# METHODS-Group/ProximalGalerkin

Hardware: AMD Instinct MI355X
Metric: proximal-Newton iterations/sec, 2048^2 P1 obstacle (LVPP Newton inner loop) (higher is better)
Workload: dtype f64; 1 GPU; 2048x2048 right-diagonal P1 obstacle problem on [-1,1]^2, phi_set obstacle, f=0, settings B: alpha double_exponential, alpha_max 100, tol 0.0001; snes_rtol 1e-6, Newton linear solves to true relative residual 1e-10; mixed_unknowns=8396802, step=one full LVPP solve from the zero state, parallelism=single

## Files before the change

### include/pgx.h

```cpp
#ifndef PGX_H
#define PGX_H

#include <stdint.h>

#ifdef __cplusplus
extern "C" {
#endif

#define PGX_OK 0
#define PGX_EINVAL (-1)
#define PGX_EHIP (-2)
#define PGX_ENODEV (-3)
#define PGX_ENOMEM (-4)
#define PGX_ESTATE (-5)
#define PGX_ECOMM (-6)

#define PGX_SNES_CONVERGED_FNORM_ABS 2
#define PGX_SNES_CONVERGED_FNORM_RELATIVE 3
#define PGX_SNES_CONVERGED_SNORM_RELATIVE 4
#define PGX_SNES_DIVERGED_LINEAR_SOLVE (-3)
#define PGX_SNES_DIVERGED_FNORM_NAN (-4)
#define PGX_SNES_DIVERGED_MAX_IT (-5)
#define PGX_SNES_DIVERGED_DTOL (-9)

// ... 85 lines not shown

int pgx_umg_level_export(pgx_handle* h, int level, int32_t* n, int32_t* nnz, int32_t* rowptr, int32_t* col, double* K, double* M, double* D,
                         uint8_t* mask);
int pgx_umg_cycle_apply(pgx_handle* h, int level, int nu, double omega, const double* b, double* z);

int pgx_p2_cycle_info(pgx_handle* h, int32_t out[8], double* patch_omega);
int pgx_p2_patch_export(pgx_handle* h, int32_t* pdof, double* Ainv);
int pgx_p2_wide_export(pgx_handle* h, int32_t* nw, int32_t* verts, int32_t* wdof, double* Ainv);
int pgx_p2_cycle_apply(pgx_handle* h, int stage, int nu, double omega, const double* b, const double* x0, double* z);

int pgx_newton_solve(pgx_handle* h, const pgx_snes_opts* opts, int* reason, int* its, int* lin_its);
int pgx_observables(pgx_handle* h, double out[6]);

int pgx_reduce_selfcheck(pgx_handle* h, int nv, int64_t len, int basis_f32, int reps, uint64_t seed, int64_t* mismatches);

int pgx_profile_enable(pgx_handle* h, int on);
int pgx_profile_get(pgx_handle* h, double ms[8], int reset);

typedef struct pgx_comm pgx_comm;

typedef struct pgx_partition {
  int32_t rank, size;
  int32_t global_ny;
  int32_t dist_levels;
} pgx_partition;

int pgx_partition_rows(pgx_partition* part, int32_t* row0, int32_t* nrows, int32_t* own0, int32_t* nown);

int pgx_comm_rccl_unique_id(char id[128]);
int pgx_comm_rccl_init(const char id[128], int rank, int size, int device, pgx_comm** out);
// ... 23 lines not shown
```

### proximalgalerkin_amd/_lib.py

```python
from __future__ import annotations

import ctypes as C
import pathlib

import numpy as np

_HERE = pathlib.Path(__file__).resolve().parent
import os as _os

LIB_PATH = pathlib.Path(_os.environ.get("PGX_LIB", _HERE / "libpgx.so"))

c_double_p = C.POINTER(C.c_double)
c_int32_p = C.POINTER(C.c_int32)
c_int64_p = C.POINTER(C.c_int64)


class PgxError(RuntimeError):
    pass


class pgx_mesh(C.Structure):
    _fields_ = [
        ("n_vertices", C.c_int32),
        ("n_cells", C.c_int32),
# ... 345 lines not shown
    ("pgx_umg_transfer_export", C.c_int, [_H, C.c_int, c_int32_p, c_int32_p, c_int32_p, c_int32_p, c_int32_p, c_double_p]),
    ("pgx_umg_level_export", C.c_int,
     [_H, C.c_int, c_int32_p, c_int32_p, c_int32_p, c_int32_p, c_double_p, c_double_p, c_double_p, C.POINTER(C.c_uint8)]),
    ("pgx_umg_cycle_apply", C.c_int, [_H, C.c_int, C.c_int, C.c_double, c_double_p, c_double_p]),
    ("pgx_p2_cycle_info", C.c_int, [_H, c_int32_p, c_double_p]),
    ("pgx_p2_patch_export", C.c_int, [_H, c_int32_p, c_double_p]),
    ("pgx_p2_wide_export", C.c_int, [_H, c_int32_p, c_int32_p, c_int32_p, c_double_p]),
    ("pgx_p2_cycle_apply", C.c_int, [_H, C.c_int, C.c_int, C.c_double, c_double_p, c_double_p, c_double_p]),
    ("pgx_spmv_select", C.c_int, [_H, C.c_int, C.POINTER(C.c_int)]),
    ("pgx_p2_stencil_info", C.c_int, [_H, C.POINTER(C.c_int32)]),
    ("pgx_comm_counts", C.c_int, [_H, C.POINTER(C.c_int64), C.c_int]),
    ("pgx_newton_solve", C.c_int,
     [_H, C.POINTER(pgx_snes_opts), C.POINTER(C.c_int), C.POINTER(C.c_int), C.POINTER(C.c_int)]),
    ("pgx_observables", C.c_int, [_H, c_double_p]),
    ("pgx_reduce_selfcheck", C.c_int, [_H, C.c_int, C.c_int64, C.c_int, C.c_int, C.c_uint64, c_int64_p]),
    ("pgx_profile_enable", C.c_int, [_H, C.c_int]),
    ("pgx_profile_get", C.c_int, [_H, c_double_p, C.c_int]),
    ("pgx_partition_rows", C.c_int,
     [C.POINTER(pgx_partition), c_int32_p, c_int32_p, c_int32_p, c_int32_p]),
    ("pgx_comm_rccl_unique_id", C.c_int, [C.c_char_p]),
    ("pgx_comm_rccl_init", C.c_int, [C.c_char_p, C.c_int, C.c_int, C.c_int, C.POINTER(_COMM)]),
    ("pgx_comm_local_group", C.c_int, [C.c_int, C.POINTER(_COMM)]),
    ("pgx_comm_shm_init", C.c_int, [C.c_char_p, C.c_int, C.c_int, C.c_uint64, C.c_int, C.POINTER(_COMM)]),
    ("pgx_comm_allreduce", C.c_int, [_COMM, c_double_p, C.c_uint64]),
    ("pgx_comm_halo", C.c_int, [_COMM, c_double_p, c_double_p] + [C.c_uint64] * 8),
    ("pgx_comm_gather0", C.c_int, [_COMM, c_double_p, C.c_uint64, c_double_p]),
    ("pgx_comm_scatter0", C.c_int, [_COMM, c_double_p, C.c_uint64, c_double_p]),
    ("pgx_comm_selfcheck", C.c_int, [_COMM, C.c_int, C.c_double]),
    ("pgx_comm_free", None, [_COMM]),
    ("pgx_comm_last_error", C.c_char_p, []),
# ... 225 lines not shown
```

### proximalgalerkin_amd/csrc/pgx_api.hip

```cpp
#include <algorithm>
#include <atomic>
#include <chrono>
#include <thread>
#include <cmath>
#include <cstdio>
#include <cstring>
#include <deque>
#include <map>
#include <mutex>
#include <string>
#include <vector>

#include "../../include/pgx.h"
#include "../../include/pgx_nd.h"
#include "pgx_comm.h"
#include "pgx_handle.h"
#include "pgx_internal.h"

static thread_local std::string g_create_error;

namespace {
std::mutex g_tune_mu;
std::atomic<int> g_tune_gen{0};
std::map<std::string, const std::string*>& tune_table() {
// ... 931 lines not shown
  if (!h->patch_f32) h->patch_sym = 0;
  if (h->patch_f32 == 2 && !h->patch_sym) h->patch_f32 = 1;
  if (const char* e = pgx_tune("PGX_P2_FALLBACK_ITS")) h->p2_fallback_its = std::max(1, atoi(e));
  {
    const char* e = pgx_tune("PGX_TAIL2");
    pgxk_mg_tail_select(e ? atoi(e) : 1);
  }
  if (const char* e = pgx_tune("PGX_FUSED_LEGS")) h->fused_legs = atoi(e);
  if (const char* e = pgx_tune("PGX_FUSED_K3")) h->fused_k3 = atoi(e);
  if (const char* e = pgx_tune("PGX_NU_COARSE")) h->nu_coarse = atoi(e);
  if (const char* e = pgx_tune("PGX_SPMV_STREAM")) h->spmv_stream = atoi(e);
  if (const char* e = pgx_tune("PGX_SPMV_BAL")) h->spmv_bal = atoi(e);
  if (const char* e = pgx_tune("PGX_SPMV_DICT")) h->spmv_dict = atoi(e);
  if (const char* e = pgx_tune("PGX_SPMV_STENCIL")) h->spmv_stencil = atoi(e);
  if (const char* e = pgx_tune("PGX_RESID_GRID")) h->resid_grid = atoi(e);
  if (const char* e = pgx_tune("PGX_D_DIRECT")) h->d_direct = atoi(e);
  if (const char* e = pgx_tune("PGX_RAP_LDS_MIN")) h->rap_lds_min = atoi(e);
  if (const char* e = pgx_tune("PGX_K6_MAX")) h->k6_max = atoi(e);
  if (const char* e = pgx_tune("PGX_SMOOTH_D32")) h->smooth_d32 = atoi(e);
  if (const char* e = pgx_tune("PGX_HOST_POLL")) h->host_poll = atoi(e);
  if (const char* e = pgx_tune("PGX_GS_WIDE")) h->gs_wide = atoi(e) >= 16 ? 16 : 8;
  if (const char* e = pgx_tune("PGX_FUSED_PUBLISH")) h->fused_publish = atoi(e);
  if (const char* e = pgx_tune("PGX_TICKET_REDUCE")) h->ticket_reduce = atoi(e);
  if (const char* e = pgx_tune("PGX_FUSED_RESID")) h->fused_resid = atoi(e);
  if (const char* e = pgx_tune("PGX_LEAN_RHS")) h->lean_rhs = atoi(e);
  if (const char* e = pgx_tune("PGX_FUSED_STEP")) h->fused_step = atoi(e);
  if (const char* e = pgx_tune("PGX_LAZY_NORM")) h->lazy_norm = atoi(e);
  if (const char* e = pgx_tune("PGX_V_F32")) h->v_f32 = atoi(e);
  if (const char* e = pgx_tune("PGX_V_F32_GAIN")) h->v_f32_gain = atof(e);
  if (const char* e = pgx_tune("PGX_V_F32_MAX")) h->v_f32_max = atof(e);
// ... 360 lines not shown
  HIPCHK(hipMemcpyAsync(dst, src, sizeof(double) * 2 * (size_t)h->nd, hipMemcpyHostToDevice, h->st));
  HIPCHK(hipStreamSynchronize(h->st));
  return PGX_OK;
}
static int copy_out(pgx_handle* h, double* dst, const double* src) {
  HIPCHK(hipMemcpyAsync(dst, src, sizeof(double) * 2 * (size_t)h->nd, hipMemcpyDeviceToHost, h->st));
  HIPCHK(hipStreamSynchronize(h->st));
  return PGX_OK;
}
extern "C" int pgx_set_state(pgx_handle* h, const double* x) {
  NEED(h);
  if (!x) return PGX_EINVAL;
  return copy_in(h, h->x, x);
}
extern "C" int pgx_get_state(pgx_handle* h, double* x) {
  NEED(h);
  if (!x) return PGX_EINVAL;
  return copy_out(h, x, h->x);
}
extern "C" int pgx_set_prev(pgx_handle* h, const double* x) {
  NEED(h);
  if (!x) return PGX_EINVAL;
  return copy_in(h, h->xk, x);
}
extern "C" int pgx_get_prev(pgx_handle* h, double* x) {
  NEED(h);
  if (!x) return PGX_EINVAL;
  return copy_out(h, x, h->xk);
}
extern "C" int pgx_advance_prev(pgx_handle* h) {
  NEED(h);
  pgxk_scale_copy(h->st, 2 * (size_t)h->nd, 1.0, h->x, h->xk);
  HIPCHK(hipStreamSynchronize(h->st));
  return PGX_OK;
}
extern "C" int pgx_zero_state(pgx_handle* h) {
  NEED(h);
  HIPCHK(hipMemsetAsync(h->x, 0, sizeof(double) * 2 * (size_t)h->nd, h->st));
  HIPCHK(hipMemsetAsync(h->xk, 0, sizeof(double) * 2 * (size_t)h->nd, h->st));
  HIPCHK(hipStreamSynchronize(h->st));
  return PGX_OK;
}
extern "C" int pgx_owned_range(const pgx_handle* h, int64_t* offset, int64_t* count) {
  if (!h) return PGX_EINVAL;
  if (offset) *offset = h->dist.on ? (int64_t)h->dist.own_off : 0;
  if (count) *count = h->dist.on ? (int64_t)h->dist.own_cnt : (int64_t)(h->degree == 2 ? h->n : h->nd);
// ... 13 lines not shown
  if (rc) return rc;
  HIPCHK(hipStreamSynchronize(h->st));
  return PGX_OK;
}
extern "C" int pgx_set_alpha(pgx_handle* h, double a) {
  if (!h || !(a > 0.0)) return PGX_EINVAL;
  h->alpha = a;
  return PGX_OK;
}

static bool d_direct_on(const pgx_handle* h) {
  return h->d_direct && !h->dist.on && h->degree == 1 && h->structured && h->resid_grid && !h->lev.empty() && h->lev[0].uniform &&
         sizeof(dsten_t) == 8 && !h->lev[0].Dh32;
}

static void residual_dev(pgx_handle* h, const double* x, double* F, int with_d = 0) {
  PhaseTimer t(h, 0);
  if (h->degree == 2) {
    pgxk_residual_p2_cells(h->st, h->nc, h->nd, h->cdofs, h->coords, h->mask, h->gbc, x, h->xk, h->alpha, h->f, h->q2,
                           h->p2_v2c_ptr, h->p2_v2c_ent, h->p2_stash, F, h->geoq);
    pgxk_residual_final(h->st, h->nd, h->mask, h->gbc, h->bphi, x, F);
    return;
  }
  if (h->resid_grid && h->structured && !h->lev.empty() && h->lev[0].uniform) {
    pgxk_resid_fill_grid(h->st, with_d ? 1 : 0, h->lev[0], h->fill_lds, h->rowptr, h->v2c_ptr, h->v2c_ent, h->v2c_pos, h->cells,
                         h->coords, h->mask, h->gbc, h->bphi, x, h->xk, h->alpha, h->f, h->q, F, h->Dv, with_d, d_direct_on(h), h->colm);
    h->dh_interior = with_d != 0;
    h->d0_direct = with_d != 0 && d_direct_on(h);
    if (with_d == 2) h->dv_lean = true;
    if (with_d == 1) h->dv_lean = false;
    return;
  }
  pgxk_resid_fill_p1(h->st, with_d, h->n, h->fill_lds, h->rowptr, h->v2c_ptr, h->v2c_ent, h->v2c_pos, h->cells,
                     h->coords, h->mask, h->gbc, h->bphi, x, h->xk, h->alpha, h->f, h->q, F, h->Dv, h->geoq);
}

static int jacobian_dev(pgx_handle* h, const double* x, bool have_d = false) {
  if (!(have_d && h->degree == 1)) {
    PhaseTimer t(h, 1);
    if (h->degree == 2) {
      pgxk_fill_rows_p2(h->st, 2, h->nd, h->s_fill_lds, h->s_rowptr, h->p2_v2c_ptr, h->p2_v2c_ent, h->p2_v2c_pos,
                        h->cdofs, h->coords, x + h->nd, h->q2, h->s_D, h->geoq);
      pgxk_fill_rows_p1_Dp2(h->st, h->n, h->fill_lds, h->rowptr, h->v2c_ptr, h->v2c_ent, h->v2c_pos, h->cdofs, h->coords,
                            x + h->nd, h->q2, h->Dv, h->geoq);
    } else if (h->resid_grid && h->structured && !h->lev.empty() && h->lev[0].uniform) {
      pgxk_resid_fill_grid(h->st, 1, h->lev[0], h->fill_lds, h->rowptr, h->v2c_ptr, h->v2c_ent, h->v2c_pos, h->cells, h->coords,
                           h->mask, h->gbc, h->bphi, x, h->xk, h->alpha, h->f, h->q, h->w, h->Dv, 1, d_direct_on(h), h->colm);
      h->dh_interior = true;
      h->d0_direct = d_direct_on(h);
      h->dv_lean = false;
      have_d = true;
    } else {
      pgxk_fill_rows(h->st, 2, h->n, h->fill_lds, h->rowptr, h->v2c_ptr, h->v2c_ent, h->v2c_pos, h->cells, h->coords,
                     x + h->n, h->q, h->Dv, h->geoq);
    }
  }
  if (h->structured) {
    PhaseTimer t(h, 2);
    const bool direct = d_direct_on(h);
    const bool d0 = direct && have_d && h->dh_interior && h->d0_direct;
// ... 1602 lines not shown
  NEED(h);
  if (h->degree == 2) {
    if (kind == 0) h->p2st.select = 0;
    else if (kind == 1 || kind == 3) h->p2st.select = 1;
    else if (kind != -1) return PGX_EINVAL;
    if (active) *active = (h->p2st.state && h->p2st.select && (!h->dist.on || h->p2st.dist_enable) && h->spmv_stream && h->spmv_bal) ? 3 : 0;
    return PGX_OK;
  }
  if (kind == 0 || kind == 1 || kind == 2) h->spmv_stencil = kind;
  else if (kind != -1) return PGX_EINVAL;
  if (active) *active = (h->spmv_stencil && h->structured && h->degree == 1) ? h->spmv_stencil : 0;
  return PGX_OK;
}

extern "C" int pgx_observables(pgx_handle* h, double out[6]) {
  NEED(h);
  if (!out) return PGX_EINVAL;
  {
    PhaseTimer t(h, 6);
    if (h->degree == 2 && !h->dist.on) {
      pgxk_observables_p2_cells(h->st, h->nc, h->nd, h->cdofs, h->coords, h->x, h->xk, h->alpha, h->f, h->q2,
                                h->obs_partials, h->obs_blocks, h->geoq);
      pgxk_observables_final(h->st, h->obs_blocks, h->obs_partials, h->d_out6);
    } else if (h->dist.on && h->degree == 2) {
      const Dist& D = h->dist;
      pgxk_observables_p2_cells(h->st, D.ncell_own, h->nd, h->cdofs + 6 * (size_t)D.cell0, h->coords, h->x, h->xk, h->alpha, h->f,
                                h->q2, h->obs_partials, pgxk_observables_blocks(D.ncell_own));
      pgxk_observables_final_raw(h->st, pgxk_observables_blocks(D.ncell_own), h->obs_partials, h->d_out6);
      const int rc = allreduce_dev(h, h->d_out6, 6);
      if (rc) return rc;
    } else if (h->dist.on) {
// ... 13 lines not shown
    if (rcb) return rcb;
  }
  {
    const int rcf = fetch_small(h, h->d_out6, 6);
    if (rcf) return rcf;
  }
  for (int k = 0; k < 6; ++k) out[k] = h->h_small[k];
  if (h->dist.on) {
    out[1] = std::fabs(out[1]);
    out[4] = std::sqrt(out[4]);
    out[5] = std::sqrt(out[5]);
  }
  return PGX_OK;
}

extern "C" int pgx_profile_enable(pgx_handle* h, int on) {
  if (!h) return PGX_EINVAL;
  h->prof = on != 0;
  return PGX_OK;
}
extern "C" int pgx_profile_get(pgx_handle* h, double ms[8], int reset) {
  if (!h || !ms) return PGX_EINVAL;
  for (int k = 0; k < 8; ++k) ms[k] = h->ms[k];
  if (reset)
    for (int k = 0; k < 8; ++k) h->ms[k] = 0.0;
  return PGX_OK;
}

extern "C" int pgx_newton_solve(pgx_handle* h, const pgx_snes_opts* opts, int* reason, int* its_out, int* lin_out) {
  NEED(h);
  if (!opts || !reason) return PGX_EINVAL;
  pgx_snes_opts optv = *opts;
  if (!(optv.ksp_rtol > 0.0)) optv.ksp_rtol = (h->degree == 2) ? 1e-11 : 1e-10;
  opts = &optv;
  const bool p2_hier = h->structured ? h->lev.size() > 1 : (umg_on(h) && h->n >= h->umg_min_p2);
  const bool mg_first = optv.pc_type == 0 && h->degree == 2 && p2_hier && h->patch_nn && h->p2_patch && !h->dist.on && !h->lu_comm;
  const bool umg_auto = h->degree == 1 && umg_on(h) && h->n >= h->umg_min;
  bool use_lu = h->lu_comm || optv.pc_type == 2 ||
                (optv.pc_type == 0 && (h->degree == 2 || !h->structured) && !h->dist.on && !mg_first && !umg_auto);
  h->lu_active = false;
  if (use_lu) {
    int rcl = ensure_lu(h);
    if (rcl) return rcl;
  }
  if (h->dist.on && h->degree == 2 && optv.ksp_max_it == 200) optv.ksp_max_it = 400;
// ... 9 lines not shown
  h->umg_idle = use_lu;
  PgxRange range("pgx:newton_solve");
  int its = 0, lin = 0, rsn = 0;
  double fnorm = 0, fnorm0 = 0, ttol = 0;
  h->omega_now = 0.0;
  h->v_f32_off = false;
  int rc = PGX_OK;
  const bool dist = h->dist.on;
  const size_t nk = dist ? 2 * h->dist.nk_field() : n2;
  auto owned_norm = [&](const double* v, double* out) -> int {
    if (!dist) return dev_norm(h, v, out);
    gather_owned(h, v, h->dist.wc);
    return dev_norm(h, h->dist.wc, out, nk);
  };
  const int with_d = (!use_lu && !mg_first && h->degree == 1 && h->structured && h->spmv_stencil == 1 && h->lean_d) ? 2 : 1;
  pgxk_scale_copy(h->st, n2, 1.0, h->x, h->xw);
  residual_dev(h, h->xw, h->F, with_d);
  if ((rc = replica_check(h, h->F, n2, "the residual"))) return rc;
  if (dist) {
    gather_owned(h, h->F, h->rhs);
    rc = dev_norm(h, h->rhs, &fnorm, nk);
  } else {
    rc = dev_norm(h, h->F, &fnorm);
  }
  if (rc) return rc;
  fnorm0 = fnorm;
  if (opts->monitor) printf("  0 SNES Function norm %.12e\n", fnorm);
  if (!std::isfinite(fnorm))
    rsn = PGX_SNES_DIVERGED_FNORM_NAN;
  else if (fnorm < opts->snes_atol)
    rsn = PGX_SNES_CONVERGED_FNORM_ABS;
  ttol = fnorm * opts->snes_rtol;
// ... 80 lines not shown
        if (rc) return rc;
        rc = owned_norm(h->xw, &xnorm);
        if (rc) return rc;
      }
      if (snorm < opts->snes_stol * xnorm)
        rsn = PGX_SNES_CONVERGED_SNORM_RELATIVE;
      else if (fnorm > opts->snes_divtol * fnorm0)
        rsn = PGX_SNES_DIVERGED_DTOL;
    }
  }
  h->lu_active = false;
  if (rsn > 0) pgxk_scale_copy(h->st, n2, 1.0, h->xw, h->x);
  if (h->dh_interior || h->dv_lean) h->jac_valid = false;
  HIPCHK(hipStreamSynchronize(h->st));
  HIPCHK(hipGetLastError());
  if (h->prof) h->ms[7] += scope.stop();
  *reason = rsn;
  if (its_out) *its_out = its;
  if (lin_out) *lin_out = lin;
  return PGX_OK;
}
```

### proximalgalerkin_amd/csrc/pgx_handle.h

```cpp
#pragma once
#include <algorithm>
#include <string>
#include <vector>

#include "../../include/pgx.h"
#include "../../include/pgx_nd.h"
#include "pgx_comm.h"
#include "pgx_internal.h"

struct DistLevel {
  int g, glo, H, ghi;
};
struct Dist {
  bool on = false;
  pgx_comm* comm = nullptr;
  int rank = 0, size = 1, ldist = 0, global_ny = 0;
  std::vector<DistLevel> L;
  GridLevel view{};
  int view_row0 = 0, view_glo = 0, view_H = 0, view_own0 = 0;
  long long n_halo = 0, n_allreduce = 0, n_vcycle = 0, n_krylov = 0;
  double* view_S = nullptr;
  size_t own_off = 0, own_cnt = 0;
  size_t eb = 0, eown_off = 0, eown_cnt = 0;
  size_t nk_field() const { return own_cnt + eown_cnt; }
// ... 146 lines not shown
  pgx_comm* lu_comm = nullptr;
  double* Jmix = nullptr;
  bool dh_interior = false;
  int d_direct = 1;
  int rap_lds_min = 60000;
  bool d0_direct = false;
  int stag_its = 12;
  double stag_gain = 1e-4;
  int smooth_d32 = 0;
  int k6_max = 0;
  int mg_f32 = 1;
  int f32_min = 4000;
  int f32_k6_max = 4300000;
  int f32_rr_max = 300000;
  int resid_grid = 1;
  int spmv_stencil = 1;
  bool lu_active = false;
  bool check_replicas = false;
  double *obs_partials = nullptr, *d_out6 = nullptr;
  int obs_blocks = 0;
  bool prof = false;
  double ms[8] = {0, 0, 0, 0, 0, 0, 0, 0};
  hipEvent_t e0 = nullptr, e1 = nullptr;
  std::vector<void*> allocs;
};

static inline bool umg_on(const pgx_handle* h) { return h->umg.size() > 1 && h->umg_enable; }

#define HIPCHK(call)                                                                           \
  do {                                                                                          \
// ... 63 lines not shown
    pgx_roctx(names[s & 7]);
    if (h->prof) hipEventRecord(h->e0, h->st);
  }
  ~PhaseTimer() {
    pgx_roctx(nullptr);
    if (h->prof) {
      hipEventRecord(h->e1, h->st);
      hipEventSynchronize(h->e1);
      float ms = 0;
      hipEventElapsedTime(&ms, h->e0, h->e1);
      h->ms[slot] += ms;
    }
  }
};

#define NEED(hh)          \
  if (!(hh)) return PGX_EINVAL; \
  hipSetDevice((hh)->device)

#pragma GCC visibility push(hidden)
int precond(pgx_handle* h, const double* b, double* z, int nu, double omega);
void spmv_dev(pgx_handle* h, const double* x, double* y);
void gather_owned(pgx_handle* h, const double* loc, double* cmp);
int allreduce_dev(pgx_handle* h, double* dev, size_t n);
bool f32_cycle_ok(const pgx_handle* h, int l, int nu);

void pgxk_amg_direct(hipStream_t st, int n, const int32_t* ptr, const int32_t* src, const double* K, double* val);
void pgxk_amg_pvalues(hipStream_t st, int n, const int32_t* fptr, const int32_t* own, const int32_t* pptr, const int32_t* pa, const int32_t* pb,
                      const int32_t* diag, const double* K, const double* p0, double trunc, double* val);
int pgx_amg_build_device(pgx_handle* h, double theta, double trunc, int32_t min_coarse, double max_keep, int32_t* n_levels, double* seconds);
void pgxk_amg_rap(hipStream_t st, const UmgLevel& C, const double* src, double* dst);
void pgxk_amg_resid_restrict(hipStream_t st, const UmgLevel& C, const double* ru, const double* rp);
void pgxk_amg_prolong_add(hipStream_t st, int n_f, const UmgLevel& C, double* xu, double* xp);
// ... 52 lines not shown
```

### proximalgalerkin_amd/csrc/pgx_internal.h

```cpp
#pragma once
#include <hip/hip_runtime.h>
#include <stdint.h>
#include <stddef.h>

#include "pgx_scope.h"

#ifdef PGX_DSTEN_FLOAT
typedef float dsten_t;
#else
typedef double dsten_t;
#endif

#define PGX_MAX_NQ 16
#define PGX_BLOCK 256
#ifndef PGX_TILE_X
#define PGX_TILE_X 32
#define PGX_TILE_Y 16
#endif
#ifndef PGX_ROWMAP_TY
#define PGX_ROWMAP_TY 16
#endif
#ifndef PGX_ROWMAP_BLOCK
#define PGX_ROWMAP_BLOCK 512
#endif
// ... 229 lines not shown
                    void* Dst, int f32);
void pgxk_p2st_check(hipStream_t st, const P2StTab& S, int nx, int nv, int i0, int ni, int j0, int nj, double alpha_ref, double tol,
                     const int32_t* rowptr, const double* K, const double* M, int* fail);
void pgxk_p2_rows_csr(hipStream_t st, int nrows, const int32_t* rows, const int32_t* rowptr, const int32_t* colm, const double* K,
                      const double* M, const double* D, double alpha, const uint8_t* mask, const double* xu, const double* xp,
                      const double* bu, const double* bp, double* yu, double* yp);
void pgxk_resid_fill_p1(hipStream_t st, int write_d, int n, size_t lds_bytes, const int32_t* rowptr,
                        const int32_t* v2c_ptr, const int32_t* v2c_ent, const int32_t* v2c_pos, const int32_t* cells,
                        const double* coords, const uint8_t* mask, const double* gbc, const double* bphi,
                        const double* x, const double* xk, double alpha, double f, QuadTab q, double* F, double* Dout,
                        const double* geo = nullptr);
void pgxk_resid_fill_grid(hipStream_t st, int write_d, const GridLevel& L, size_t lds_bytes, const int32_t* rowptr,
                          const int32_t* v2c_ptr, const int32_t* v2c_ent, const int32_t* v2c_pos, const int32_t* cells,
                          const double* coords, const uint8_t* mask, const double* gbc, const double* bphi, const double* x,
                          const double* xk, double alpha, double f, QuadTab q, double* F, double* Dout, int write_sh,
                          int direct = 0, const int32_t* colm = nullptr);
void pgxk_multiaxpy_scale(hipStream_t st, size_t len, int nv, const double* V, size_t ldv, const double* h,
                          double scale, double* w);
bool pgxk_multiaxpy_norm(hipStream_t st, size_t len, int nv, const double* V, size_t ldv, const double* h, double* w,
                         double* partials, double* out, int wide = 8, PgxTicket* tk = nullptr);
bool pgxk_multiaxpy_norm_f32(hipStream_t st, size_t len, int nv, const float* V, size_t ldv, const double* h, int from_vnext, double* w,
                             float* vnext, double* partials, double* out, int wide = 8, PgxTicket* tk = nullptr);
void pgxk_f_pack_d(hipStream_t st, const GridLevel& L);
void pgxk_f_smooth(hipStream_t st, int K, int first, const GridLevel& L, double alpha, const float2* xf, const double* b64u,
                   const double* b64p, const GridLevel* C, const float2* cf, const double* cdu, const double* cdp, double omega,
                   int remap, float2* yf, double* y64u, double* y64p, float2* cbf = nullptr, double* cb64u = nullptr,
                   double* cb64p = nullptr, double bscale = 1.0,
                   const float* b32u = nullptr, const float* b32p = nullptr);
void pgxk_f_resid_restrict(hipStream_t st, const GridLevel& L, double alpha, const float2* xf, const GridLevel& C, int remap,
                           float2* cbf, double* cb64u, double* cb64p);
int pgxk_st_smooth6_ok(const GridLevel& L);
// ... 4 lines not shown
```

### proximalgalerkin_amd/csrc/pgx_kernels.hip

```cpp
#include "pgx_internal.h"
#include "pgx_stencil.h"
#include <algorithm>
#include <type_traits>

#define WAVE 64

static bool first_use_on_device(int slot) {
  static bool done[4][64] = {};
  int dev = 0;
  if (hipGetDevice(&dev) != hipSuccess || dev < 0 || dev >= 64) return true;
  if (done[slot][dev]) return false;
  done[slot][dev] = true;
  return true;
}

__device__ __forceinline__ double wave_sum(double v) {
#pragma unroll
  for (int o = WAVE / 2; o > 0; o >>= 1) v += __shfl_xor(v, o, WAVE);
  return v;
}

__device__ __forceinline__ double2 ldnt2(const double2* p) {
  typedef double v2d __attribute__((ext_vector_type(2)));
  const v2d v = __builtin_nontemporal_load((const v2d*)p);
// ... 413 lines not shown
      }
    }
    F[i] = mask[i] ? x[i] - gbc[i] : Fu;
    F[n + i] = Fp - bphi[i];
    if (WRITE_D && FRAME)
      for (int k = rowptr[i]; k < rowptr[i + 1]; ++k) Dout[k] = row[k - rowptr[i]];
  }
  if (WRITE_D && !FRAME) {
    __syncthreads();
    for (int k = threadIdx.x; k < len; k += PGX_BLOCK) Dout[base + k] = acc[k];
  }
}

#define PGX_RF_TX 32
#define PGX_RF_TY 12
template <bool WRITE_D>
__global__ void __launch_bounds__(PGX_RF_TX * PGX_RF_TY) k_resid_fill_grid(
    int nx, int ny, int n, const int32_t* __restrict__ rowptr, const double* __restrict__ coords, const uint8_t* __restrict__ mask,
    const double* __restrict__ gbc, const double* __restrict__ bphi, const double* __restrict__ x, const double* __restrict__ xk,
    double alpha, double f, QuadTab q, StConst sc, double* __restrict__ F, double* __restrict__ Dout,
    dsten_t* __restrict__ Sh, double4* __restrict__ Dd4, void* __restrict__ Dq, int dbf16) {
  constexpr int TX = PGX_RF_TX, TY = PGX_RF_TY, IW = TX + 2, IH = TY + 2, SW = TX + 1, SH = TY + 1;
  __shared__ double iu[IH * IW], ip[IH * IW], idp[IH * IW];
  __shared__ double E[2 * SW * SH][6];
  const int sx = nx + 1;
  const int ntx = (nx - 1 + TX - 1) / TX;
  const int i1 = 1 + ((int)blockIdx.x % ntx) * TX, j1 = 1 + ((int)blockIdx.x / ntx) * TY;
  const int tid = threadIdx.x;
  for (int t = tid; t < IH * IW; t += TX * TY) {
    const int gi = i1 - 1 + t % IW, gj = j1 - 1 + t / IW;
    double u = 0.0, p = 0.0, dp = 0.0;
    if (gi <= nx && gj <= ny) {
      const int v = gj * sx + gi;
      u = mask[v] ? gbc[v] : x[v];
      p = x[n + v];
      dp = p - xk[n + v];
    }
    iu[t] = u;
    ip[t] = p;
    idp[t] = dp;
  }
  __syncthreads();
  for (int t = tid; t < 2 * SW * SH; t += TX * TY) {
    const int sq = t >> 1, a = sq % SW, b = sq / SW;
    double e[6] = {0.0, 0.0, 0.0, 0.0, 0.0, 0.0};
    if (i1 - 1 + a < nx && j1 - 1 + b < ny) {
      const int o = b * IW + a;
      const double p0 = ip[o], p1 = (t & 1) ? ip[o + IW + 1] : ip[o + 1], p2 = (t & 1) ? ip[o + IW] : ip[o + IW + 1];
      for (int k = 0; k < q.nq; ++k) {
        const double n0 = q.N[k][0], n1 = q.N[k][1], n2 = q.N[k][2];
        const double w = q.w[k] * exp(p0 * n0 + p1 * n1 + p2 * n2);
        e[0] += w * n0 * n0;
        e[1] += w * n1 * n1;
        e[2] += w * n2 * n2;
        e[3] += w * n0 * n1;
        e[4] += w * n0 * n2;
        e[5] += w * n1 * n2;
// ... 166 lines not shown
                         bphi, x, xk, alpha, f, q, F, Dout, geo);
    return;
  }
  if (write_d)
    hipLaunchKernelGGL((k_resid_fill_p1<true, false>), grid, block, lds_bytes, st, n, rowptr, v2c_ptr, v2c_ent, v2c_pos, cells,
                       coords, mask, gbc, bphi, x, xk, alpha, f, q, 0, 0, F, Dout);
  else
    hipLaunchKernelGGL((k_resid_fill_p1<false, false>), grid, block, lds_bytes, st, n, rowptr, v2c_ptr, v2c_ent, v2c_pos, cells,
                       coords, mask, gbc, bphi, x, xk, alpha, f, q, 0, 0, F, Dout);
}

void pgxk_resid_fill_grid(hipStream_t st, int write_d, const GridLevel& L, size_t lds_bytes, const int32_t* rowptr,
                          const int32_t* v2c_ptr, const int32_t* v2c_ent, const int32_t* v2c_pos, const int32_t* cells,
                          const double* coords, const uint8_t* mask, const double* gbc, const double* bphi, const double* x,
                          const double* xk, double alpha, double f, QuadTab q, double* F, double* Dout, int write_sh, int direct,
                          const int32_t* colm) {
  const int n = L.n, sx = L.nx + 1;
  const bool copies = direct && write_d && write_sh && colm;
  double4* Dd4 = copies ? L.Dd4 : nullptr;
  void* Dq = copies && L.f32 ? L.Dq : nullptr;
  if (direct && colm) {
    const int nframe = 2 * sx + 2 * (L.ny - 1);
    dim3 grid((nframe + PGX_FRAME_BLOCK - 1) / PGX_FRAME_BLOCK), block(PGX_FRAME_BLOCK);
    if (write_d)
      hipLaunchKernelGGL(k_resid_fill_frame<true>, grid, block, 0, st, L.nx, L.ny, n, rowptr, colm, v2c_ptr, v2c_ent, v2c_pos, cells,
                         coords, mask, gbc, bphi, x, xk, alpha, f, q, F, Dout, copies ? L.Dh : nullptr, Dd4, Dq, L.dbf16);
    else
      hipLaunchKernelGGL(k_resid_fill_frame<false>, grid, block, 0, st, L.nx, L.ny, n, rowptr, colm, v2c_ptr, v2c_ent, v2c_pos, cells,
                         coords, mask, gbc, bphi, x, xk, alpha, f, q, F, Dout, nullptr, nullptr, nullptr, 0);
  } else {
    dim3 grid((n + PGX_BLOCK - 1) / PGX_BLOCK), block(PGX_BLOCK);
    if (write_d)
      hipLaunchKernelGGL((k_resid_fill_p1<true, true>), grid, block, lds_bytes, st, n, rowptr, v2c_ptr, v2c_ent, v2c_pos, cells,
                         coords, mask, gbc, bphi, x, xk, alpha, f, q, sx, L.ny, F, Dout);
    else
      hipLaunchKernelGGL((k_resid_fill_p1<false, true>), grid, block, lds_bytes, st, n, rowptr, v2c_ptr, v2c_ent, v2c_pos, cells,
                         coords, mask, gbc, bphi, x, xk, alpha, f, q, sx, L.ny, F, Dout);
  }
  if (L.nx < 2 || L.ny < 2) return;
  const int ntx = (L.nx - 1 + PGX_RF_TX - 1) / PGX_RF_TX, nty = (L.ny - 1 + PGX_RF_TY - 1) / PGX_RF_TY;
  const StConst sc = make_stconst(L);
  if (write_d)
    hipLaunchKernelGGL(k_resid_fill_grid<true>, dim3(ntx * nty), dim3(PGX_RF_TX * PGX_RF_TY), 0, st, L.nx, L.ny, n, rowptr, coords,
                       mask, gbc, bphi, x, xk, alpha, f, q, sc, F, write_sh == 2 ? nullptr : Dout, write_sh ? L.Dh : nullptr, Dd4, Dq,
                       L.dbf16);
  else
    hipLaunchKernelGGL(k_resid_fill_grid<false>, dim3(ntx * nty), dim3(PGX_RF_TX * PGX_RF_TY), 0, st, L.nx, L.ny, n, rowptr, coords,
                       mask, gbc, bphi, x, xk, alpha, f, q, sc, F, Dout, nullptr, nullptr, nullptr, 0);
}

void pgxk_fill_rows(hipStream_t st, int mode, int n, size_t lds_bytes, const int32_t* rowptr, const int32_t* v2c_ptr,
                    const int32_t* v2c_ent, const int32_t* v2c_pos, const int32_t* cells, const double* coords,
                    const double* psi, QuadTab q, double* out, const double* geo) {
  dim3 grid((n + PGX_BLOCK - 1) / PGX_BLOCK), block(PGX_BLOCK);
  if (geo) {
    if (mode == 0)
      hipLaunchKernelGGL(k_fill_rows_c<0>, grid, block, lds_bytes, st, n, rowptr, v2c_ptr, v2c_ent, v2c_pos, cells, psi, q, out, geo);
// ... 3199 lines not shown
```

### proximalgalerkin_amd/problem.py

```python
from __future__ import annotations

import ctypes as C
import warnings
from dataclasses import dataclass

import numpy as np

from . import _lib
from .fem import Constant, DirichletBC, Function, QuadratureFunction

SNES_CONVERGED_FNORM_ABS = 2
SNES_CONVERGED_FNORM_RELATIVE = 3
SNES_CONVERGED_SNORM_RELATIVE = 4
SNES_DIVERGED_LINEAR_SOLVE = -3
SNES_DIVERGED_FNORM_NAN = -4
SNES_DIVERGED_MAX_IT = -5
SNES_DIVERGED_DTOL = -9


class ConvergenceError(RuntimeError):
    """Raised for snes_error_if_not_converged / ksp_error_if_not_converged (obstacle_pg.py:132,135)."""


@dataclass
# ... 453 lines not shown
                         "pgx_p2_cycle_apply")
        return z

    def observables(self):
        self._sync_inputs()
        out = np.empty(6)
        _lib.check(self._lib, self._h, self._lib.pgx_observables(self._h, _lib.dptr(out)), "pgx_observables")
        return out

    def reduce_selfcheck(self, nv, length, basis_f32=False, reps=1, seed=0):
        bad = C.c_int64(-1)
        _lib.check(self._lib, self._h, self._lib.pgx_reduce_selfcheck(self._h, int(nv), int(length), int(bool(basis_f32)), int(reps),
                                                                      int(seed), C.byref(bad)), "pgx_reduce_selfcheck")
        return bad.value

    def owned_edge_range(self):
        off, cnt = C.c_int64(0), C.c_int64(0)
        _lib.check(self._lib, self._h, self._lib.pgx_owned_edge_range(self._h, C.byref(off), C.byref(cnt)),
                   "pgx_owned_edge_range")
        return off.value, cnt.value

    def owned_range(self):
        off, cnt = C.c_int64(0), C.c_int64(0)
        _lib.check(self._lib, self._h, self._lib.pgx_owned_range(self._h, C.byref(off), C.byref(cnt)),
                   "pgx_owned_range")
        return off.value, cnt.value

    def profile(self, enable=None, reset=False):
        if enable is not None:
            self._lib.pgx_profile_enable(self._h, int(enable))
# ... 54 lines not shown
```

Baseline: 160.4 Newton iterations/s.

## Skip Jacobian-data refill in first residual after converged Newton solve

When a new Newton solve starts right after a converged one on the same state, the entry residual launches a reduced grid kernel. That kernel computes only the u-block residual from a 7-point stencil and reuses the psi residual and the Jacobian D/stencil buffers kept from the last solve. A freshness stamp records which flags those buffers were built under, and any API call that may change inputs invalidates it. This removes the heavy nonlinear element pass at solve entry. The price is a state-tracking invariant that must stay correct, and a selfcheck API is added to verify bitwise agreement with the full path.

After: 162.2 Newton iterations/s, median of 6. +1.1%, better.

```diff
diff --git a/include/pgx.h b/include/pgx.h
--- a/include/pgx.h
+++ b/include/pgx.h
@@ -123,6 +123,9 @@
 
 int pgx_reduce_selfcheck(pgx_handle* h, int nv, int64_t len, int basis_f32, int reps, uint64_t seed, int64_t* mismatches);
 
+int pgx_resid_reuse_counts(pgx_handle* h, int64_t out[2], int reset);
+int pgx_resid_reuse_selfcheck(pgx_handle* h, int64_t out[6]);
+
 int pgx_profile_enable(pgx_handle* h, int on);
 int pgx_profile_get(pgx_handle* h, double ms[8], int reset);
 
diff --git a/proximalgalerkin_amd/_lib.py b/proximalgalerkin_amd/_lib.py
--- a/proximalgalerkin_amd/_lib.py
+++ b/proximalgalerkin_amd/_lib.py
@@ -383,6 +383,8 @@
      [_H, C.POINTER(pgx_snes_opts), C.POINTER(C.c_int), C.POINTER(C.c_int), C.POINTER(C.c_int)]),
     ("pgx_observables", C.c_int, [_H, c_double_p]),
     ("pgx_reduce_selfcheck", C.c_int, [_H, C.c_int, C.c_int64, C.c_int, C.c_int, C.c_uint64, c_int64_p]),
+    ("pgx_resid_reuse_counts", C.c_int, [_H, c_int64_p, C.c_int]),
+    ("pgx_resid_reuse_selfcheck", C.c_int, [_H, c_int64_p]),
     ("pgx_profile_enable", C.c_int, [_H, C.c_int]),
     ("pgx_profile_get", C.c_int, [_H, c_double_p, C.c_int]),
     ("pgx_partition_rows", C.c_int,
diff --git a/proximalgalerkin_amd/csrc/pgx_api.hip b/proximalgalerkin_amd/csrc/pgx_api.hip
--- a/proximalgalerkin_amd/csrc/pgx_api.hip
+++ b/proximalgalerkin_amd/csrc/pgx_api.hip
@@ -969,6 +969,7 @@
   if (const char* e = pgx_tune("PGX_SPMV_DICT")) h->spmv_dict = atoi(e);
   if (const char* e = pgx_tune("PGX_SPMV_STENCIL")) h->spmv_stencil = atoi(e);
   if (const char* e = pgx_tune("PGX_RESID_GRID")) h->resid_grid = atoi(e);
+  if (const char* e = pgx_tune("PGX_RESID_REUSE")) h->resid_reuse = atoi(e);
   if (const char* e = pgx_tune("PGX_D_DIRECT")) h->d_direct = atoi(e);
   if (const char* e = pgx_tune("PGX_RAP_LDS_MIN")) h->rap_lds_min = atoi(e);
   if (const char* e = pgx_tune("PGX_K6_MAX")) h->k6_max = atoi(e);
@@ -1359,22 +1360,22 @@
   return copy_in(h, h->x, x);
 }
 extern "C" int pgx_get_state(pgx_handle* h, double* x) {
-  NEED(h);
+  NEED_KEEP(h);
   if (!x) return PGX_EINVAL;
   return copy_out(h, x, h->x);
 }
 extern "C" int pgx_set_prev(pgx_handle* h, const double* x) {
-  NEED(h);
+  NEED_KEEP(h);
   if (!x) return PGX_EINVAL;
   return copy_in(h, h->xk, x);
 }
 extern "C" int pgx_get_prev(pgx_handle* h, double* x) {
-  NEED(h);
+  NEED_KEEP(h);
   if (!x) return PGX_EINVAL;
   return copy_out(h, x, h->xk);
 }
 extern "C" int pgx_advance_prev(pgx_handle* h) {
-  NEED(h);
+  NEED_KEEP(h);
   pgxk_scale_copy(h->st, 2 * (size_t)h->nd, 1.0, h->x, h->xk);
   HIPCHK(hipStreamSynchronize(h->st));
   return PGX_OK;
@@ -1418,7 +1419,15 @@
          sizeof(dsten_t) == 8 && !h->lev[0].Dh32;
 }
 
-static void residual_dev(pgx_handle* h, const double* x, double* F, int with_d = 0) {
+static bool resid_grid_on(const pgx_handle* h) {
+  return h->degree == 1 && h->resid_grid && h->structured && !h->lev.empty() && h->lev[0].uniform;
+}
+
+static bool resid_reuse_on(const pgx_handle* h) {
+  return h->resid_reuse && resid_grid_on(h) && !h->dist.on && !h->lu_comm && h->mg_f32;
+}
+
+static void residual_dev(pgx_handle* h, const double* x, double* F, int with_d = 0, bool fu_only = false) {
   PhaseTimer t(h, 0);
   if (h->degree == 2) {
     pgxk_residual_p2_cells(h->st, h->nc, h->nd, h->cdofs, h->coords, h->mask, h->gbc, x, h->xk, h->alpha, h->f, h->q2,
@@ -1426,9 +1435,10 @@
     pgxk_residual_final(h->st, h->nd, h->mask, h->gbc, h->bphi, x, F);
     return;
   }
-  if (h->resid_grid && h->structured && !h->lev.empty() && h->lev[0].uniform) {
+  if (resid_grid_on(h)) {
     pgxk_resid_fill_grid(h->st, with_d ? 1 : 0, h->lev[0], h->fill_lds, h->rowptr, h->v2c_ptr, h->v2c_ent, h->v2c_pos, h->cells,
-                         h->coords, h->mask, h->gbc, h->bphi, x, h->xk, h->alpha, h->f, h->q, F, h->Dv, with_d, d_direct_on(h), h->colm);
+                         h->coords, h->mask, h->gbc, h->bphi, x, h->xk, h->alpha, h->f, h->q, F, h->Dv, with_d, d_direct_on(h), h->colm,
+                         fu_only ? 1 : 0);
     h->dh_interior = with_d != 0;
     h->d0_direct = with_d != 0 && d_direct_on(h);
     if (with_d == 2) h->dv_lean = true;
@@ -1447,7 +1457,7 @@
                         h->cdofs, h->coords, x + h->nd, h->q2, h->s_D, h->geoq);
       pgxk_fill_rows_p1_Dp2(h->st, h->n, h->fill_lds, h->rowptr, h->v2c_ptr, h->v2c_ent, h->v2c_pos, h->cdofs, h->coords,
                             x + h->nd, h->q2, h->Dv, h->geoq);
-    } else if (h->resid_grid && h->structured && !h->lev.empty() && h->lev[0].uniform) {
+    } else if (resid_grid_on(h)) {
       pgxk_resid_fill_grid(h->st, 1, h->lev[0], h->fill_lds, h->rowptr, h->v2c_ptr, h->v2c_ent, h->v2c_pos, h->cells, h->coords,
                            h->mask, h->gbc, h->bphi, x, h->xk, h->alpha, h->f, h->q, h->w, h->Dv, 1, d_direct_on(h), h->colm);
       h->dh_interior = true;
@@ -3080,7 +3090,7 @@
 }
 
 extern "C" int pgx_observables(pgx_handle* h, double out[6]) {
-  NEED(h);
+  NEED_KEEP(h);
   if (!out) return PGX_EINVAL;
   {
     PhaseTimer t(h, 6);
@@ -3124,6 +3134,72 @@
   return PGX_OK;
 }
 
+extern "C" int pgx_resid_reuse_counts(pgx_handle* h, int64_t out[2], int reset) {
+  if (!h || !out) return PGX_EINVAL;
+  out[0] = h->entry_full;
+  out[1] = h->entry_reduced;
+  if (reset) h->entry_full = h->entry_reduced = 0;
+  return PGX_OK;
+}
+
+extern "C" int pgx_resid_reuse_selfcheck(pgx_handle* h, int64_t out[6]) {
+  if (!h) return PGX_EINVAL;
+  const pgx_handle::ResidFresh fr = h->fresh;
+  NEED(h);
+  if (!out) return PGX_EINVAL;
+  if (!(resid_reuse_on(h) && fr.valid && fr.dh_interior == h->dh_interior && fr.d0_direct == h->d0_direct && fr.dv_lean == h->dv_lean)) {
+    h->err = "pgx_resid_reuse_selfcheck: no valid stamp (call it after a converged pgx_newton_solve of a handle PGX_RESID_REUSE applies to)";
+    return PGX_EINVAL;
+  }
+  const GridLevel& L = h->lev[0];
+  const size_t n = (size_t)h->n;
+  struct Buf {
+    const void* dev;
+    size_t bytes;
+  };
+  const Buf bufs[5] = {{h->F + n, n * sizeof(double)},
+                       {L.Dh, 4 * n * sizeof(dsten_t)},
+                       {L.Dd4, L.Dd4 ? n * sizeof(double4) : 0},
+                       {L.Dq, (L.f32 && L.Dq) ? n * (L.dbf16 ? sizeof(uint2) : sizeof(float4)) : 0},
+                       {h->Dv, h->Dv ? (size_t)h->nnz * sizeof(double) : 0}};
+  using Snap = std::vector<std::vector<unsigned char>>;
+  auto snapshot = [&](Snap& s) -> int {
+    s.resize(5);
+    for (int k = 0; k < 5; ++k) {
+      s[k].resize(bufs[k].bytes);
+      if (bufs[k].bytes) HIPCHK(hipMemcpyAsync(s[k].data(), bufs[k].dev, bufs[k].bytes, hipMemcpyDeviceToHost, h->st));
+    }
+    HIPCHK(hipStreamSynchronize(h->st));
+    return PGX_OK;
+  };
+  auto differing = [](const std::vector<unsigned char>& a, const std::vector<unsigned char>& b, size_t word) {
+    int64_t c = 0;
+    for (size_t i = 0; i < a.size(); i += word) c += memcmp(a.data() + i, b.data() + i, word) != 0;
+    return c;
+  };
+  Snap held, after_reduced, after_full;
+  std::vector<double> fu_reduced(n), fu_full(n);
+  int rc = snapshot(held);
+  if (rc) return rc;
+  residual_dev(h, h->x, h->F, fr.with_d, true);
+  HIPCHK(hipMemcpyAsync(fu_reduced.data(), h->F, n * sizeof(double), hipMemcpyDeviceToHost, h->st));
+  if ((rc = snapshot(after_reduced))) return rc;
+  residual_dev(h, h->x, h->F, fr.with_d, false);
+  HIPCHK(hipMemcpyAsync(fu_full.data(), h->F, n * sizeof(double), hipMemcpyDeviceToHost, h->st));
+  if ((rc = snapshot(after_full))) return rc;
+  HIPCHK(hipGetLastError());
+  out[0] = 0;
+  for (size_t i = 0; i < n; ++i) out[0] += memcmp(&fu_reduced[i], &fu_full[i], sizeof(double)) != 0;
+  out[1] = differing(held[0], after_reduced[0], sizeof(double));
+  out[2] = 0;
+  for (int k = 1; k < 5; ++k) out[2] += differing(held[k], after_reduced[k], 8);
+  out[3] = differing(held[0], after_full[0], sizeof(double));
+  out[4] = 0;
+  for (int k = 1; k < 5; ++k) out[4] += differing(held[k], after_full[k], 8);
+  out[5] = (int64_t)n;
+  return PGX_OK;
+}
+
 extern "C" int pgx_profile_enable(pgx_handle* h, int on) {
   if (!h) return PGX_EINVAL;
   h->prof = on != 0;
@@ -3138,7 +3214,7 @@
 }
 
 extern "C" int pgx_newton_solve(pgx_handle* h, const pgx_snes_opts* opts, int* reason, int* its_out, int* lin_out) {
-  NEED(h);
+  NEED_KEEP(h);
   if (!opts || !reason) return PGX_EINVAL;
   pgx_snes_opts optv = *opts;
   if (!(optv.ksp_rtol > 0.0)) optv.ksp_rtol = (h->degree == 2) ? 1e-11 : 1e-10;
@@ -3178,8 +3254,13 @@
     return dev_norm(h, h->dist.wc, out, nk);
   };
   const int with_d = (!use_lu && !mg_first && h->degree == 1 && h->structured && h->spmv_stencil == 1 && h->lean_d) ? 2 : 1;
+  const bool reuse_ok = resid_reuse_on(h) && !use_lu;
+  const bool fu_only = reuse_ok && h->fresh.valid && h->fresh.with_d == with_d && h->fresh.dh_interior == h->dh_interior &&
+                       h->fresh.d0_direct == h->d0_direct && h->fresh.dv_lean == h->dv_lean;
+  h->fresh.valid = false;
+  ++(fu_only ? h->entry_reduced : h->entry_full);
   pgxk_scale_copy(h->st, n2, 1.0, h->x, h->xw);
-  residual_dev(h, h->xw, h->F, with_d);
+  residual_dev(h, h->xw, h->F, with_d, fu_only);
   if ((rc = replica_check(h, h->F, n2, "the residual"))) return rc;
   if (dist) {
     gather_owned(h, h->F, h->rhs);
@@ -3290,6 +3371,7 @@
   if (h->dh_interior || h->dv_lean) h->jac_valid = false;
   HIPCHK(hipStreamSynchronize(h->st));
   HIPCHK(hipGetLastError());
+  if (rsn > 0 && reuse_ok && h->dh_interior) h->fresh = {true, with_d, h->dh_interior, h->d0_direct, h->dv_lean};
   if (h->prof) h->ms[7] += scope.stop();
   *reason = rsn;
   if (its_out) *its_out = its;
diff --git a/proximalgalerkin_amd/csrc/pgx_handle.h b/proximalgalerkin_amd/csrc/pgx_handle.h
--- a/proximalgalerkin_amd/csrc/pgx_handle.h
+++ b/proximalgalerkin_amd/csrc/pgx_handle.h
@@ -184,6 +184,13 @@
   int f32_k6_max = 4300000;
   int f32_rr_max = 300000;
   int resid_grid = 1;
+  int resid_reuse = 1;
+  struct ResidFresh {
+    bool valid = false;
+    int with_d = 0;
+    bool dh_interior = false, d0_direct = false, dv_lean = false;
+  } fresh;
+  int64_t entry_full = 0, entry_reduced = 0;
   int spmv_stencil = 1;
   bool lu_active = false;
   bool check_replicas = false;
@@ -277,9 +284,12 @@
   }
 };
 
-#define NEED(hh)          \
+#define NEED_KEEP(hh)          \
   if (!(hh)) return PGX_EINVAL; \
   hipSetDevice((hh)->device)
+#define NEED(hh)  \
+  NEED_KEEP(hh);  \
+  (hh)->fresh.valid = false
 
 #pragma GCC visibility push(hidden)
 int precond(pgx_handle* h, const double* b, double* z, int nu, double omega);
diff --git a/proximalgalerkin_amd/csrc/pgx_internal.h b/proximalgalerkin_amd/csrc/pgx_internal.h
--- a/proximalgalerkin_amd/csrc/pgx_internal.h
+++ b/proximalgalerkin_amd/csrc/pgx_internal.h
@@ -267,7 +267,7 @@
                           const int32_t* v2c_ptr, const int32_t* v2c_ent, const int32_t* v2c_pos, const int32_t* cells,
                           const double* coords, const uint8_t* mask, const double* gbc, const double* bphi, const double* x,
                           const double* xk, double alpha, double f, QuadTab q, double* F, double* Dout, int write_sh,
-                          int direct = 0, const int32_t* colm = nullptr);
+                          int direct = 0, const int32_t* colm = nullptr, int fu_only = 0);
 void pgxk_multiaxpy_scale(hipStream_t st, size_t len, int nv, const double* V, size_t ldv, const double* h,
                           double scale, double* w);
 bool pgxk_multiaxpy_norm(hipStream_t st, size_t len, int nv, const double* V, size_t ldv, const double* h, double* w,
diff --git a/proximalgalerkin_amd/csrc/pgx_kernels.hip b/proximalgalerkin_amd/csrc/pgx_kernels.hip
--- a/proximalgalerkin_amd/csrc/pgx_kernels.hip
+++ b/proximalgalerkin_amd/csrc/pgx_kernels.hip
@@ -451,15 +451,15 @@
 
 #define PGX_RF_TX 32
 #define PGX_RF_TY 12
-template <bool WRITE_D>
+template <bool WRITE_D, bool FU_ONLY = false>
 __global__ void __launch_bounds__(PGX_RF_TX * PGX_RF_TY) k_resid_fill_grid(
     int nx, int ny, int n, const int32_t* __restrict__ rowptr, const double* __restrict__ coords, const uint8_t* __restrict__ mask,
     const double* __restrict__ gbc, const double* __restrict__ bphi, const double* __restrict__ x, const double* __restrict__ xk,
     double alpha, double f, QuadTab q, StConst sc, double* __restrict__ F, double* __restrict__ Dout,
     dsten_t* __restrict__ Sh, double4* __restrict__ Dd4, void* __restrict__ Dq, int dbf16) {
   constexpr int TX = PGX_RF_TX, TY = PGX_RF_TY, IW = TX + 2, IH = TY + 2, SW = TX + 1, SH = TY + 1;
-  __shared__ double iu[IH * IW], ip[IH * IW], idp[IH * IW];
-  __shared__ double E[2 * SW * SH][6];
+  __shared__ double iu[IH * IW], ip[FU_ONLY ? 1 : IH * IW], idp[IH * IW];
+  __shared__ double E[FU_ONLY ? 1 : 2 * SW * SH][6];
   const int sx = nx + 1;
   const int ntx = (nx - 1 + TX - 1) / TX;
   const int i1 = 1 + ((int)blockIdx.x % ntx) * TX, j1 = 1 + ((int)blockIdx.x / ntx) * TY;
@@ -474,10 +474,27 @@
       dp = p - xk[n + v];
     }
     iu[t] = u;
-    ip[t] = p;
+    if (!FU_ONLY) ip[t] = p;
     idp[t] = dp;
   }
   __syncthreads();
+  if (FU_ONLY) {
+    const int li = tid % TX, lj = tid / TX, gi = i1 + li, gj = j1 + lj;
+    if (gi >= nx || gj >= ny) return;
+    const int v = gj * sx + gi;
+    const double adet = fabs((coords[2] - coords[0]) * (coords[2 * sx + 1] - coords[1]));
+    const int o = (lj + 1) * IW + li + 1;
+    const int off[7] = {0, 1, -1, IW, -IW, IW + 1, -IW - 1};
+    double Ku = 0.0, Mdp = 0.0;
+#pragma unroll
+    for (int t = 0; t < 7; ++t) {
+      Ku += sc.K[t] * iu[o + off[t]];
+      Mdp += sc.M[t] * idp[o + off[t]];
+    }
+    const double load = adet * 2.0 * (q.mref[0] + q.mref[1] + q.mref[2]);
+    F[v] = mask[v] ? x[v] - gbc[v] : alpha * Ku + Mdp - alpha * f * load;
+    return;
+  }
   for (int t = tid; t < 2 * SW * SH; t += TX * TY) {
     const int sq = t >> 1, a = sq % SW, b = sq / SW;
     double e[6] = {0.0, 0.0, 0.0, 0.0, 0.0, 0.0};
@@ -674,7 +691,7 @@
                           const int32_t* v2c_ptr, const int32_t* v2c_ent, const int32_t* v2c_pos, const int32_t* cells,
                           const double* coords, const uint8_t* mask, const double* gbc, const double* bphi, const double* x,
                           const double* xk, double alpha, double f, QuadTab q, double* F, double* Dout, int write_sh, int direct,
-                          const int32_t* colm) {
+                          const int32_t* colm, int fu_only) {
   const int n = L.n, sx = L.nx + 1;
   const bool copies = direct && write_d && write_sh && colm;
   double4* Dd4 = copies ? L.Dd4 : nullptr;
@@ -700,7 +717,10 @@
   if (L.nx < 2 || L.ny < 2) return;
   const int ntx = (L.nx - 1 + PGX_RF_TX - 1) / PGX_RF_TX, nty = (L.ny - 1 + PGX_RF_TY - 1) / PGX_RF_TY;
   const StConst sc = make_stconst(L);
-  if (write_d)
+  if (fu_only)
+    hipLaunchKernelGGL((k_resid_fill_grid<false, true>), dim3(ntx * nty), dim3(PGX_RF_TX * PGX_RF_TY), 0, st, L.nx, L.ny, n, rowptr,
+                       coords, mask, gbc, bphi, x, xk, alpha, f, q, sc, F, nullptr, nullptr, nullptr, nullptr, 0);
+  else if (write_d)
     hipLaunchKernelGGL(k_resid_fill_grid<true>, dim3(ntx * nty), dim3(PGX_RF_TX * PGX_RF_TY), 0, st, L.nx, L.ny, n, rowptr, coords,
                        mask, gbc, bphi, x, xk, alpha, f, q, sc, F, write_sh == 2 ? nullptr : Dout, write_sh ? L.Dh : nullptr, Dd4, Dq,
                        L.dbf16);
diff --git a/proximalgalerkin_amd/problem.py b/proximalgalerkin_amd/problem.py
--- a/proximalgalerkin_amd/problem.py
+++ b/proximalgalerkin_amd/problem.py
@@ -491,6 +491,17 @@
                                                                       int(seed), C.byref(bad)), "pgx_reduce_selfcheck")
         return bad.value
 
+    def resid_reuse_counts(self, reset=False):
+        out = (C.c_int64 * 2)()
+        _lib.check(self._lib, self._h, self._lib.pgx_resid_reuse_counts(self._h, out, int(reset)), "pgx_resid_reuse_counts")
+        return int(out[0]), int(out[1])
+
+    def resid_reuse_selfcheck(self):
+        self._sync_inputs()
+        out = (C.c_int64 * 6)()
+        _lib.check(self._lib, self._h, self._lib.pgx_resid_reuse_selfcheck(self._h, out), "pgx_resid_reuse_selfcheck")
+        return [int(v) for v in out]
+
     def owned_edge_range(self):
         off, cnt = C.c_int64(0), C.c_int64(0)
         _lib.check(self._lib, self._h, self._lib.pgx_owned_edge_range(self._h, C.byref(off), C.byref(cnt)),
```
